# quziyan/NPairLoss

Measured on NVIDIA H100. Metric: N-pair fwd+bwd samples/sec at B=8192,D=512, higher is better.
Workload: dtype f32 (3-pass fp16-split wgmma, f32 accumulate)

## Files before the change

### npairloss_b200/csrc/kernels.cu

```cuda
#include <cassert>
#include <cstdlib>
#include "device.cuh"
#include "kernels.cuh"
#include <cuda.h>

#include <cuda_bf16.h>
#include <cuda_fp16.h>
#include <cfloat>

#include "thresholds.cuh"

namespace npair {
unsigned long long g_kernel_launches = 0;


__device__ __forceinline__ float fast_exp_m2(float sv, float m2) {
  float y;
  asm("ex2.approx.ftz.f32 %0, %1;" : "=f"(y) : "f"(fmaf(sv, LOG2E, -m2)));
  return y;
}

template <bool VEC>
__device__ __forceinline__ float4 load4(const float* __restrict__ x, long long q) {
  if (VEC) return __ldg(reinterpret_cast<const float4*>(x) + q);
  return make_float4(__ldg(x + 4 * q), __ldg(x + 4 * q + 1), __ldg(x + 4 * q + 2), __ldg(x + 4 * q + 3));
}
template <bool VEC>
__device__ __forceinline__ void abs_sum_max(const float* __restrict__ x, long long n, long long t0, long long stride, bool want_max,
                                            float& sum, float& mx) {
  const long long n4 = n >> 2;
  long long i = t0;
  for (; i + 3 * stride < n4; i += 4 * stride) {
    const float4 a = load4<VEC>(x, i), b = load4<VEC>(x, i + stride), c = load4<VEC>(x, i + 2 * stride), d = load4<VEC>(x, i + 3 * stride);
    const float a0 = fabsf(a.x), a1 = fabsf(a.y), a2 = fabsf(a.z), a3 = fabsf(a.w), b0 = fabsf(b.x), b1 = fabsf(b.y), b2 = fabsf(b.z), b3 = fabsf(b.w);
    const float c0 = fabsf(c.x), c1 = fabsf(c.y), c2 = fabsf(c.z), c3 = fabsf(c.w), d0 = fabsf(d.x), d1 = fabsf(d.y), d2 = fabsf(d.z), d3 = fabsf(d.w);
    sum += (a0 + a1) + (a2 + a3) + (b0 + b1) + (b2 + b3) + (c0 + c1) + (c2 + c3) + (d0 + d1) + (d2 + d3);
    if (want_max) {
      mx = fmaxf(mx, fmaxf(fmaxf(fmaxf(a0, a1), fmaxf(a2, a3)), fmaxf(fmaxf(b0, b1), fmaxf(b2, b3))));
      mx = fmaxf(mx, fmaxf(fmaxf(fmaxf(c0, c1), fmaxf(c2, c3)), fmaxf(fmaxf(d0, d1), fmaxf(d2, d3))));
    }
  }
  for (; i < n4; i += stride) {
    const float4 a = load4<VEC>(x, i);
    sum += (fabsf(a.x) + fabsf(a.y)) + (fabsf(a.z) + fabsf(a.w));
    if (want_max) mx = fmaxf(mx, fmaxf(fmaxf(fabsf(a.x), fabsf(a.y)), fmaxf(fabsf(a.z), fabsf(a.w))));
  }
  for (long long j = (n4 << 2) + t0; j < n; j += stride) { sum += fabsf(x[j]); if (want_max) mx = fmaxf(mx, fabsf(x[j])); }
}
template <bool DISJOINT = false>
__device__ __forceinline__ bool prep_reduce_body(const float* __restrict__ xl, long long nl, const float* __restrict__ xt, long long ntot,
                                                 float* __restrict__ partial, int want_scale, RowArrays ra, int Q, BlockScalars* bs) {
  __shared__ float s_sum[8], s_max[8];
  __shared__ int s_last;
  float sum = 0.f, mx = 0.f;
  const long long stride = static_cast<long long>(gridDim.x) * blockDim.x;
  const long long t0 = static_cast<long long>(blockIdx.x) * blockDim.x + threadIdx.x;
  const bool same_range = !DISJOINT && want_scale && xl == xt && nl == ntot;
  const bool local_max = DISJOINT ? want_scale != 0 : same_range;
  if ((reinterpret_cast<uintptr_t>(xl) & 15) == 0) abs_sum_max<true>(xl, nl, t0, stride, local_max, sum, mx);
  else abs_sum_max<false>(xl, nl, t0, stride, local_max, sum, mx);
  if (want_scale && !same_range) {
    if ((reinterpret_cast<uintptr_t>(xt) & 15) == 0) {
      const float4* x4 = reinterpret_cast<const float4*>(xt);
      const long long n4 = ntot >> 2;
      long long i = t0;
      for (; i + 3 * stride < n4; i += 4 * stride) {
        const float4 a = __ldg(x4 + i), b = __ldg(x4 + i + stride), c = __ldg(x4 + i + 2 * stride), d = __ldg(x4 + i + 3 * stride);
        mx = fmaxf(mx, fmaxf(fmaxf(fmaxf(fabsf(a.x), fabsf(a.y)), fmaxf(fabsf(a.z), fabsf(a.w))), fmaxf(fmaxf(fabsf(b.x), fabsf(b.y)), fmaxf(fabsf(b.z), fabsf(b.w)))));
        mx = fmaxf(mx, fmaxf(fmaxf(fmaxf(fabsf(c.x), fabsf(c.y)), fmaxf(fabsf(c.z), fabsf(c.w))), fmaxf(fmaxf(fabsf(d.x), fabsf(d.y)), fmaxf(fabsf(d.z), fabsf(d.w)))));
      }
      for (; i < n4; i += stride) { const float4 a = __ldg(x4 + i); mx = fmaxf(mx, fmaxf(fmaxf(fabsf(a.x), fabsf(a.y)), fmaxf(fabsf(a.z), fabsf(a.w)))); }
      for (long long j = (n4 << 2) + t0; j < ntot; j += stride) mx = fmaxf(mx, fabsf(xt[j]));
    } else {
      for (long long i = t0; i < ntot; i += stride) mx = fmaxf(mx, fabsf(xt[i]));
    }
  }
  for (long long i = t0; i < Q; i += stride) reset_row_stats(ra, i);
  sum = warp_sum(sum); mx = warp_max(mx);
  const int w = threadIdx.x >> 5, l = threadIdx.x & 31;
  if (l == 0) { s_sum[w] = sum; s_max[w] = mx; }
  __syncthreads();
  if (threadIdx.x == 0) {
    sum = 0.f; mx = 0.f;
    for (int k = 0; k < (blockDim.x >> 5); ++k) { sum += s_sum[k]; mx = fmaxf(mx, s_max[k]); }
    partial[blockIdx.x] = sum; partial[1024 + blockIdx.x] = mx;
    __threadfence();
    s_last = (atomicAdd(&bs->ticket0, 1u) == gridDim.x - 1) ? 1 : 0;
  }
  __syncthreads();
  if (!s_last) return false;
  __threadfence();
  __shared__ double s_dsum[8];
  double dsum = 0.0; mx = 0.f;
  for (int b = threadIdx.x; b < static_cast<int>(gridDim.x); b += blockDim.x) { dsum += __ldcg(&partial[b]); mx = fmaxf(mx, __ldcg(&partial[1024 + b])); }
#pragma unroll
  for (int o = 16; o > 0; o >>= 1) { dsum += __shfl_xor_sync(0xffffffffu, dsum, o); mx = fmaxf(mx, __shfl_xor_sync(0xffffffffu, mx, o)); }
  if (l == 0) { s_dsum[w] = dsum; s_max[w] = mx; }
  __syncthreads();
  if (threadIdx.x == 0) {
    dsum = 0.0; mx = 0.f;
    for (int k = 0; k < (blockDim.x >> 5); ++k) { dsum += s_dsum[k]; mx = fmaxf(mx, s_max[k]); }
    bs->asum = static_cast<float>(dsum);
    bs->x_absmax = mx;
    float sc = 1.f, inv = 1.f;
    if (want_scale) { const PreScale ps = pre_scale(mx); sc = ps.scale; inv = ps.inv; }
    bs->x_scale = sc; bs->x_inv_scale = inv;
    bs->err = 0; bs->ticket = 0; bs->ticket2 = 0; bs->ticket0 = 0; bs->ticket3 = 0; bs->sel_active[0] = 0; bs->sel_active[1] = 0;
    bs->cand_n[0] = 0; bs->cand_n[1] = 0;
    bs->n_same = 0; bs->n_diff = 0;
  }
  return true;
}
__global__ void __launch_bounds__(256) prep_reduce_kernel(const float* __restrict__ xl, long long nl, const float* __restrict__ xt, long long ntot,
                                                          float* __restrict__ partial, int want_scale, RowArrays ra, int Q, BlockScalars* bs) {
  prep_reduce_body(xl, nl, xt, ntot, partial, want_scale, ra, Q, bs);
}
void launch_prep_reduce(const float* x_local, long long n_local, const float* x_total, long long n_total, float* partial,
                        int want_scale, RowArrays ra, int Q, BlockScalars* bs, cudaStream_t st) {
  long long nmax = n_local > n_total ? n_local : n_total;
  int nb = static_cast<int>((nmax + 256 * 16 - 1) / (256 * 16));
  if (nb < 1) nb = 1; if (nb > 592) nb = 592;
  prep_reduce_kernel<<<nb, 256, 0, st>>>(x_local, n_local, x_total, n_total, partial, want_scale, ra, Q, bs);
  count_launch();
}
__global__ void __launch_bounds__(256) prep_reduce_memory_kernel(const float* __restrict__ xl, long long nl, const float* __restrict__ xm,
                                                                 long long nm, float* __restrict__ partial, int want_scale, RowArrays ra, int Q,
                                                                 BlockScalars* bs) {
  prep_reduce_body<true>(xl, nl, xm, nm, partial, want_scale, ra, Q, bs);
}
void launch_prep_reduce_memory(const float* x_local, long long n_local, const float* x_mem, long long n_mem, float* partial, int want_scale,
                               RowArrays ra, int Q, BlockScalars* bs, cudaStream_t st) {
  int nb = static_cast<int>((n_local + n_mem + 256 * 16 - 1) / (256 * 16));
  if (nb < 1) nb = 1; if (nb > 592) nb = 592;
  prep_reduce_memory_kernel<<<nb, 256, 0, st>>>(x_local, n_local, x_mem, n_mem, partial, want_scale, ra, Q, bs);
  count_launch();
}

struct SplitArgs {
  const float* x; int N, D;
  uint16_t* Xs; long long ldXs; uint16_t* XsT; long long ldXsT; uint16_t* XlT; long long ldXlT; int row0, Q;
  uint16_t *XcatA, *XcatB; long long Dp;
};
__device__ __forceinline__ void split_load(const SplitArgs& a, int tile_d, int tile_n, float (&v)[8]) {
  const float* __restrict__ x = a.x; const int N = a.N, D = a.D;
  const int t = threadIdx.x, nl = t >> 3, dg = t & 7;
  const int n = tile_n * 32 + nl, d = tile_d * 64 + 8 * dg;
  const bool rowok = n < N;
  if (rowok && d + 7 < D && (D & 3) == 0 && (reinterpret_cast<uintptr_t>(x) & 15) == 0) {
    const float4 a4 = *reinterpret_cast<const float4*>(x + static_cast<long long>(n) * D + d);
    const float4 b4 = *reinterpret_cast<const float4*>(x + static_cast<long long>(n) * D + d + 4);
    v[0] = a4.x; v[1] = a4.y; v[2] = a4.z; v[3] = a4.w; v[4] = b4.x; v[5] = b4.y; v[6] = b4.z; v[7] = b4.w;
  } else {
#pragma unroll
    for (int e = 0; e < 8; ++e) v[e] = (rowok && d + e < D) ? x[static_cast<long long>(n) * D + d + e] : 0.f;
  }
}
template <int PREC>
__device__ __forceinline__ void split_tile(const SplitArgs& a, float sc, int tile_d, int tile_n, const float (&v)[8], int buf) {
  const int N = a.N, D = a.D;
  uint16_t* __restrict__ Xs = a.Xs; const long long ldXs = a.ldXs; uint16_t* __restrict__ XsT = a.XsT; const long long ldXsT = a.ldXsT;
  uint16_t* __restrict__ XlT = a.XlT; const long long ldXlT = a.ldXlT; const int row0 = a.row0, Q = a.Q;
  uint16_t* __restrict__ XcatA = a.XcatA; uint16_t* __restrict__ XcatB = a.XcatB; const long long Dp = a.Dp;
  constexpr int NS = SPLIT_FORMATS[PREC].pieces;
  __shared__ __align__(16) uint16_t tile2[2][NS][64][40];
  uint16_t (*tile)[64][40] = tile2[buf];
  const int n0 = tile_n * 32, d0 = tile_d * 64;
  const int t = threadIdx.x, nl = t >> 3, dg = t & 7;
  const int n = n0 + nl, d = d0 + 8 * dg;
  uint16_t p[8][3];
  uint4 pk[3];
  const bool rowok = n < N;
  split8<PREC>(v, sc, p, pk);
#pragma unroll
  for (int s = 0; s < NS; ++s)
#pragma unroll
    for (int e = 0; e < 8; ++e) tile[s][8 * dg + e][nl] = p[e][s];
  if (rowok && d < Dp && Xs) {
    const long long ps = static_cast<long long>(N) * ldXs;
#pragma unroll
    for (int s = 0; s < NS; ++s) *reinterpret_cast<uint4*>(Xs + s * ps + static_cast<long long>(n) * ldXs + d) = pk[s];
  }
  if (PREC != PREC_BF16 && XcatA && d < Dp) {
    const SimLayout L{NS, Dp};
    if (n < L.padded_rows(N)) store_sim_row<PREC>(XcatB, Dp, n, d, pk, true);
    if (n >= row0 && n < row0 + L.padded_rows(Q)) {
      uint4 pa[3];
#pragma unroll
      for (int s = 0; s < 3; ++s) pa[s] = n < row0 + Q ? pk[s] : make_uint4(0u, 0u, 0u, 0u);
      store_sim_row<PREC>(XcatA, Dp, n - row0, d, pa, false);
    }
  }
  __syncthreads();
  const int dl = t >> 2, nc = t & 3;
  const int dd = d0 + dl, nn = n0 + 8 * nc;
  if (dd < D && nn < N) {
    const long long pt = static_cast<long long>(D) * ldXsT;
    const long long pl = static_cast<long long>(D) * ldXlT;
#pragma unroll
    for (int s = 0; s < NS; ++s) {
      const uint4 q = *reinterpret_cast<const uint4*>(&tile[s][dl][8 * nc]);
      *reinterpret_cast<uint4*>(XsT + s * pt + static_cast<long long>(dd) * ldXsT + nn) = q;
      if (XlT && nn >= row0 && nn < row0 + Q) {
        if (((nn - row0) & 7) == 0 && nn + 8 <= row0 + Q) *reinterpret_cast<uint4*>(XlT + s * pl + static_cast<long long>(dd) * ldXlT + (nn - row0)) = q;
        else
          for (int e = 0; e < 8; ++e)
            if (nn + e < row0 + Q && nn + e < N) XlT[s * pl + static_cast<long long>(dd) * ldXlT + (nn + e - row0)] = tile[s][dl][8 * nc + e];
      } else if (XlT && nn < row0 && nn + 8 > row0) {
        for (int e = 0; e < 8; ++e)
          if (nn + e >= row0 && nn + e < row0 + Q && nn + e < N) XlT[s * pl + static_cast<long long>(dd) * ldXlT + (nn + e - row0)] = tile[s][dl][8 * nc + e];
      }
    }
  }
}
template <int PREC>
__global__ void __launch_bounds__(256) split_kernel(SplitArgs a, const BlockScalars* __restrict__ bs) {
  float v[8];
  split_load(a, blockIdx.x, blockIdx.y, v);
  split_tile<PREC>(a, (PREC == PREC_FP16X2) ? bs->x_scale : 1.f, blockIdx.x, blockIdx.y, v, 0);
}
__device__ __forceinline__ void split_load_memory(const SplitArgs& a, const float* __restrict__ xm, int tile_d, int tile_n, float (&v)[8]) {
  const int N = a.N, D = a.D;
  const int t = threadIdx.x, nl = t >> 3, dg = t & 7;
  const int n = tile_n * 32 + nl, d = tile_d * 64 + 8 * dg;
  const bool rowok = n < N;
  const float* x = n < a.Q ? a.x + static_cast<long long>(n) * D : xm + static_cast<long long>(n - a.Q) * D;
  if (rowok && d + 7 < D && (reinterpret_cast<uintptr_t>(x) & 15) == 0) {
    const float4 a4 = *reinterpret_cast<const float4*>(x + d);
    const float4 b4 = *reinterpret_cast<const float4*>(x + d + 4);
    v[0] = a4.x; v[1] = a4.y; v[2] = a4.z; v[3] = a4.w; v[4] = b4.x; v[5] = b4.y; v[6] = b4.z; v[7] = b4.w;
  } else {
#pragma unroll
    for (int e = 0; e < 8; ++e) v[e] = (rowok && d + e < D) ? x[d + e] : 0.f;
  }
}
template <int PREC>
__global__ void __launch_bounds__(256) split_memory_kernel(SplitArgs a, const float* __restrict__ xm, const BlockScalars* __restrict__ bs) {
  float v[8];
  split_load_memory(a, xm, blockIdx.x, blockIdx.y, v);
  split_tile<PREC>(a, (PREC == PREC_FP16X2) ? bs->x_scale : 1.f, blockIdx.x, blockIdx.y, v, 0);
}
void launch_split_memory(const float* x, int Q, const float* x_mem, int N, int D, int prec, const BlockScalars* bs, uint16_t* Xs,
                         long long ldXs, uint16_t* XsT, long long ldXsT, uint16_t* XcatA, uint16_t* XcatB, long long Dp, cudaStream_t st) {
  dim3 grid((D + 63) / 64, (N + 31) / 32);
  const SplitArgs a{x, N, D, Xs, ldXs, XsT, ldXsT, nullptr, 0, 0, Q, XcatA, XcatB, Dp};
  with_prec(prec, [&](auto P) { split_memory_kernel<P><<<grid, 256, 0, st>>>(a, x_mem, bs); });
  count_launch();
}
__global__ void memory_rows_kernel(const float* __restrict__ label, int Q, const float* __restrict__ mem_label, int m,
                                   float* __restrict__ lab_total, RowRecord* __restrict__ rec) {
  const int stride = gridDim.x * blockDim.x;
  for (int i = blockIdx.x * blockDim.x + threadIdx.x; i < Q + m; i += stride) {
    if (i < Q) { lab_total[i] = label[i]; continue; }
    const float l = mem_label[i - Q];
    lab_total[i] = l;
    rec[i] = RowRecord::memory(l);
  }
}
void launch_memory_rows(const float* label, int Q, const float* mem_label, int m, float* lab_total, RowRecord* rec, cudaStream_t st) {
  const int blocks = (Q + m + 255) / 256;
  memory_rows_kernel<<<blocks < 1024 ? blocks : 1024, 256, 0, st>>>(label, Q, mem_label, m, lab_total, rec);
  count_launch();
}

void launch_split(const float* x_total, int N, int D, int prec, const BlockScalars* bs, uint16_t* Xs, long long ldXs,
                  uint16_t* XsT, long long ldXsT, uint16_t* XlT, long long ldXlT, int row0_local, int Q,
                  uint16_t* XcatA, uint16_t* XcatB, long long Dp, cudaStream_t st) {
  dim3 grid((D + 63) / 64, (N + 31) / 32);
  const SplitArgs a{x_total, N, D, Xs, ldXs, XsT, ldXsT, XlT, ldXlT, row0_local, Q, XcatA, XcatB, Dp};
  with_prec(prec, [&](auto P) { split_kernel<P><<<grid, 256, 0, st>>>(a, bs); });
  count_launch();
}

__global__ void row_stats_ref_kernel(const __grid_constant__ SimRows sim, RowArrays ra) {
  const int i = sim.row0 + blockIdx.x;
  const float li = __ldg(sim.lab_rows + i);
  float minw = FLT_MAX, maxw = -FLT_MAX, maxb = -FLT_MAX, maxall = -FLT_MAX;
  int cnt = 0;
  const float* row = sim.row(i);
  for (int j = threadIdx.x; j < sim.N; j += blockDim.x) {
    if (j == sim.self_col(i)) continue;
    const float v = __ldg(row + j);
    maxall = fmaxf(maxall, v);
    if (__ldg(sim.lab_cols + j) == li) { minw = fminf(minw, v); maxw = fmaxf(maxw, v); ++cnt; } else maxb = fmaxf(maxb, v);
  }
  minw = warp_min(minw); maxw = warp_max(maxw); maxb = warp_max(maxb); maxall = warp_max(maxall); cnt = warp_sum_i(cnt);
  if ((threadIdx.x & 31) == 0) {
    atomicMin(&ra.st_minw[i], f2ord(minw)); atomicMax(&ra.st_maxw[i], f2ord(maxw));
    atomicMax(&ra.st_maxb[i], f2ord(maxb)); atomicMax(&ra.st_maxall[i], f2ord(maxall));
    if (cnt) atomicAdd(&ra.cnt_same[i], cnt);
  }
}
void launch_row_stats_ref(SimRows sim, RowArrays ra, cudaStream_t st) {
  row_stats_ref_kernel<<<sim.rows, 256, 0, st>>>(sim, ra);
  count_launch();
}

__global__ void __launch_bounds__(1024) thresholds_kernel(RowArrays ra, int Q, int N, MiningParams mp, BlockScalars* bs) {
  __shared__ __align__(8) unsigned char scratch[THRESHOLDS_SCRATCH_BYTES];
  thresholds_one_block(ra, Q, N, mp, bs, scratch, nullptr);
}
__global__ void thresholds_world_kernel(const BlockStats* __restrict__ xall, int xstride, int world, long long N, MiningParams mp,
                                        BlockScalars* bs) {
  if (threadIdx.x != 0 || blockIdx.x != 0) return;
  finish_thresholds(xall, world, xstride, static_cast<unsigned long long>(N), N, mp, bs);
}
void launch_thresholds_world(const float* xall, int xstride, int world, long long N, MiningParams mp, BlockScalars* bs, cudaStream_t st) {
  thresholds_world_kernel<<<1, 32, 0, st>>>(reinterpret_cast<const BlockStats*>(xall), xstride, world, N, mp, bs);
  count_launch();
}
void launch_thresholds(RowArrays ra, int Q, int N, MiningParams mp, BlockScalars* bs, cudaStream_t st) {
  thresholds_kernel<<<1, 1024, 0, st>>>(ra, Q, N, mp, bs);
  count_launch();
}

__device__ __forceinline__ float retrieval_cut(float maxw, float max_all, int lane) {
  const float pstar = expf(maxw - max_all);
  if (!(pstar > 0.f)) return -INFINITY;
  uint32_t base = f2ord(maxw), last_ok = base;
  for (int it = 0; it < 8; ++it) {
    const uint32_t kc = base - static_cast<uint32_t>(lane);
    const bool ok = (kc <= base) && (expf(ord2f(kc) - max_all) >= pstar);
    const unsigned bal = __ballot_sync(0xffffffffu, ok);
    const int T = (bal == 0xffffffffu) ? 32 : (__ffs(~bal) - 1);
    if (T > 0) last_ok = base - static_cast<uint32_t>(T - 1);
    if (T < 32) return ord2f(last_ok);
    if (base < 64u) return ord2f(last_ok);
    base -= 32u;
  }
  uint32_t lo = f2ord(-FLT_MAX), hi = last_ok;
  while (lo < hi) {
    const uint32_t mid = lo + ((hi - lo) >> 1);
    if (expf(ord2f(mid) - max_all) >= pstar) hi = mid; else lo = mid + 1u;
  }
  return ord2f(hi);
}

__device__ __forceinline__ float4 ldg_stream(const float4* p) {
  float4 v;
  asm volatile("ld.global.nc.L1::no_allocate.v4.f32 {%0, %1, %2, %3}, [%4];" : "=f"(v.x), "=f"(v.y), "=f"(v.z), "=f"(v.w) : "l"(p));
  return v;
}

__device__ __forceinline__ void lse_elem(float sv, float lab, float li, float scut, float m2, float sgn_p, float thr_p,
                                         float sgn_n, float thr_n, float& A, float& T, int& c) {
  c += (sv >= scut) ? 1 : 0;
  const float e = fast_exp_m2(sv, m2);
  const bool same = (lab == li);
  const float key = sv * (same ? sgn_p : sgn_n);
  const float es = (key <= (same ? thr_p : thr_n)) ? e : 0.f;
  T += es;
  if (same) A += es;
}

__device__ __forceinline__ void publish_tops(const TopSums* recs, int n, long long stride, long long rows, int num_tops, TopsBlock* out,
                                             unsigned int seq) {
  double ls = recs[0].loss_sum, asum = recs[0].asum;
  long long h[3] = {recs[0].hits[0], recs[0].hits[1], recs[0].hits[2]};
  int err = recs[0].err;
  for (int r = 1; r < n; ++r) {
    const TopSums& t = rank_record(recs, stride, r);
    ls += t.loss_sum; h[0] += t.hits[0]; h[1] += t.hits[1]; h[2] += t.hits[2]; asum += t.asum; err |= t.err;
  }
  float tops[5] = {0.f, 0.f, 0.f, 0.f, 0.f};
  tops[0] = static_cast<float>(ls) / static_cast<float>(-rows);
  for (int t = 1; t <= num_tops - 2 && t <= 3; ++t) tops[t] = static_cast<float>(h[t - 1]) / static_cast<float>(rows);
  tops[num_tops - 1] = static_cast<float>(asum) / static_cast<float>(rows);
  for (int t = 0; t < 5; ++t) out->tops[t] = tops[t];
  out->err = err;
  __threadfence_system();
  *reinterpret_cast<volatile unsigned int*>(&out->seq) = seq;
}

__device__ __forceinline__ void lse_finalize_block(int Q, RowArrays ra, BlockScalars* bs, int num_tops, TopsBlock* __restrict__ tops,
                                                   TopSums* __restrict__ xout, unsigned int seq, const float* __restrict__ anchor_w) {
  const int lane = threadIdx.x & 31;
  __shared__ double s_l[8];
  __shared__ int s_h[3][8];
  double ls = 0.0; int h[3] = {0, 0, 0};
  constexpr int FU = 8;
  for (int r0 = threadIdx.x; r0 < Q; r0 += FU * blockDim.x) {
    float lv[FU]; int h0[FU], h1[FU], h2[FU];
#pragma unroll
    for (int u = 0; u < FU; ++u) {
      const int r = r0 + u * blockDim.x;
      const bool ok = r < Q;
      lv[u] = ok ? __ldcg(&ra.logv[r]) : 0.f;
      if (anchor_w) {
        const float wv = ok ? __ldg(&anchor_w[r]) : 0.f;
        lv[u] = wv == 0.f ? 0.f : lv[u] * wv;
      }
      h0[u] = ok ? __ldcg(&ra.hits[r]) : 0; h1[u] = ok ? __ldcg(&ra.hits[Q + r]) : 0; h2[u] = ok ? __ldcg(&ra.hits[2 * Q + r]) : 0;
    }
#pragma unroll
    for (int u = 0; u < FU; ++u) { ls += lv[u]; h[0] += h0[u]; h[1] += h1[u]; h[2] += h2[u]; }
  }
#pragma unroll
  for (int o = 16; o > 0; o >>= 1) {
    ls += __shfl_xor_sync(0xffffffffu, ls, o);
    h[0] += __shfl_xor_sync(0xffffffffu, h[0], o); h[1] += __shfl_xor_sync(0xffffffffu, h[1], o); h[2] += __shfl_xor_sync(0xffffffffu, h[2], o);
  }
  const int w = threadIdx.x >> 5;
  if (lane == 0) { s_l[w] = ls; s_h[0][w] = h[0]; s_h[1][w] = h[1]; s_h[2][w] = h[2]; }
  __syncthreads();
  if (threadIdx.x == 0) {
    TopSums s{0.0, {0, 0, 0}, bs->asum, __ldcg(&bs->err)};
    for (int k = 0; k < (blockDim.x >> 5); ++k) { s.loss_sum += s_l[k]; s.hits[0] += s_h[0][k]; s.hits[1] += s_h[1][k]; s.hits[2] += s_h[2][k]; }
    bs->ticket = 0;
    if (xout) *xout = s;
    else publish_tops(&s, 1, 0, Q, num_tops, tops, seq);
  }
}

#ifndef NPAIR_LSE_U
#define NPAIR_LSE_U 4
#endif
#ifndef NPAIR_LSE_MINB
#define NPAIR_LSE_MINB 3
#endif
__global__ void __launch_bounds__(256, NPAIR_LSE_MINB) lse_rows_kernel(const __grid_constant__ SimRows sim, MiningParams mp, RowArrays ra, BlockScalars* bs,
                                                       int num_tops, TopsBlock* __restrict__ tops,
                                                       float m2c_off , float wscale ,
                                                       TopSums* __restrict__ xout ,
                                                       int wpr ,
                                                       unsigned int seq , int finalize,
                                                       const float* __restrict__ anchor_w , float* __restrict__ row_loss ) {
  const int lane = threadIdx.x & 31;
  __shared__ float s_pA[8], s_pT[8];
  __shared__ int s_pc[8];
#ifndef NPAIR_LSE_REV
#define NPAIR_LSE_REV 1
#endif
  const int blk = NPAIR_LSE_REV ? static_cast<int>(gridDim.x - 1 - blockIdx.x) : static_cast<int>(blockIdx.x);
  const int wib = threadIdx.x >> 5;
  const int il = blk * ((blockDim.x >> 5) / wpr) + wib / wpr;
  const int i = sim.row0 + il;
  const int Q = sim.Q, N = sim.N;
  const float* lab_cols = sim.lab_cols;
  const int part = wib % wpr;
  float A = 0.f, T = 0.f; int c = 0;
  float m2 = 0.f, thr_p = 0.f, thr_n = 0.f, li = 0.f; int cs = 0;
  if (il < sim.rows) {
    constexpr int U = NPAIR_LSE_U;
    const float* row = sim.row(i);
    const int seg = ((N + wpr - 1) / wpr + 128 * U - 1) / (128 * U) * (128 * U);
    const int c_lo = min(N, part * seg), c_hi = min(N, c_lo + seg);
    const int n_full = c_lo + (c_hi - c_lo) / (128 * U) * (128 * U);
    const float4* srow4 = reinterpret_cast<const float4*>(row + c_lo) + lane;
    const float4* lab4 = reinterpret_cast<const float4*>(lab_cols + c_lo) + lane;
    const bool lab_aligned = (reinterpret_cast<uintptr_t>(lab_cols) & 15) == 0;
    const bool fast = lab_aligned && c_lo < n_full;
    float4 v[U], vn[U];
    if (fast) {
#pragma unroll
      for (int u = 0; u < U; ++u) v[u] = ldg_stream(srow4 + 32 * u);
    }
    li = __ldg(sim.lab_rows + i);
    const int self_col = sim.self_col(i);
    const float max_all = ord2f(ra.st_maxall[i]);
    m2 = max_all * LOG2E;
    const float posi = mp.ap_region == REGION_GLOBAL ? bs->posi_global : ra.posi_thr[i];
    const float nega = mp.an_region == REGION_GLOBAL ? bs->nega_global : ra.nega_thr[i];
    if (lane == 0 && part == 0) { ra.posi_thr[i] = posi; ra.nega_thr[i] = nega; }
    const float tp = posi + mp.margin_ident;
    const float tn = nega + mp.margin_diff;
    const float sgn_p = ap_sign(mp.ap_method), sgn_n = an_sign(mp.an_method);
    thr_p = ap_thr(tp, mp.ap_method); thr_n = an_thr(tn, mp.an_method);
    cs = ra.cnt_same[i];
    const float scut = cs > 0 ? retrieval_cut(ord2f(ra.st_maxw[i]), max_all, lane) : INFINITY;
    int base = c_lo;
    if (fast) {
      for (; base < n_full; base += 128 * U, srow4 += 32 * U, lab4 += 32 * U) {
        const bool more = base + 128 * U < n_full;
        if (more) {
#pragma unroll
          for (int u = 0; u < U; ++u) vn[u] = ldg_stream(srow4 + 32 * U + 32 * u);
        }
        float4 l[U];
#pragma unroll
        for (int u = 0; u < U; ++u) l[u] = __ldg(lab4 + 32 * u);
#pragma unroll
        for (int u = 0; u < U; ++u) {
          const int j4 = base + u * 128 + lane * 4;
          const float vv[4] = {v[u].x, v[u].y, v[u].z, v[u].w};
          const float ll[4] = {l[u].x, l[u].y, l[u].z, l[u].w};
          const bool no_self = !sim.self_in4(i, j4);
          if (no_self && ll[0] != li && ll[1] != li && ll[2] != li && ll[3] != li) {
#pragma unroll
            for (int q = 0; q < 4; ++q) {
              c += (vv[q] >= scut) ? 1 : 0;
              const float e = fast_exp_m2(vv[q], m2);
              if (vv[q] * sgn_n <= thr_n) T += e;
            }
          } else if (no_self) {
#pragma unroll
            for (int q = 0; q < 4; ++q) lse_elem(vv[q], ll[q], li, scut, m2, sgn_p, thr_p, sgn_n, thr_n, A, T, c);
          } else {
#pragma unroll
            for (int q = 0; q < 4; ++q)
              if (j4 + q != self_col) lse_elem(vv[q], ll[q], li, scut, m2, sgn_p, thr_p, sgn_n, thr_n, A, T, c);
          }
        }
        if (more) {
#pragma unroll
          for (int u = 0; u < U; ++u) v[u] = vn[u];
        }
      }
    }
    for (; base < c_hi; base += 512) {
#pragma unroll 1
      for (int u = 0; u < 4; ++u) {
        const int j4 = base + u * 128 + lane * 4;
        if (j4 >= c_hi) continue;
        const float4 v4 = *reinterpret_cast<const float4*>(row + j4);
        const float vv[4] = {v4.x, v4.y, v4.z, v4.w};
#pragma unroll
        for (int q = 0; q < 4; ++q)
          if (j4 + q < c_hi && j4 + q != self_col) lse_elem(vv[q], lab_cols[j4 + q], li, scut, m2, sgn_p, thr_p, sgn_n, thr_n, A, T, c);
      }
    }
    A = warp_sum(A); T = warp_sum(T); c = warp_sum_i(c);
  }
  if (wpr > 1) {
    if (lane == 0) { s_pA[wib] = A; s_pT[wib] = T; s_pc[wib] = c; }
    __syncthreads();
    if (part == 0) {
      A = 0.f; T = 0.f; c = 0;
      for (int q = 0; q < wpr; ++q) { A += s_pA[wib + q]; T += s_pT[wib + q]; c += s_pc[wib + q]; }
    }
  }
  if (il < sim.rows && part == 0) {
    if (lane == 0) {
      ra.A[i] = A; ra.T[i] = T;
      const float lv = (A == 0.f || T == 0.f) ? 0.f : logf(A / T);
      ra.logv[i] = lv;
      if (row_loss) row_loss[i] = -lv;
      const int lim = N - 2;
      ra.hits[i] = (cs > 0 && c <= min(1, lim)) ? 1 : 0;
      ra.hits[Q + i] = (cs > 0 && c <= min(5, lim)) ? 1 : 0;
      ra.hits[2 * Q + i] = (cs > 0 && c <= min(10, lim)) ? 1 : 0;
      const float invA = A == 0.f ? 0.f : 1.f / A;
      const float invT = T == 0.f ? 0.f : 1.f / T;
      const float cA = invT - invA;
      const float amin = A > 0.f ? A : T;
      const int j = amin > 0.f ? max(0, ilogbf(wscale) - 127 - ilogbf(amin)) : 0;
      const float fsc = ldexpf(wscale, -j);
      float m2c = T == 0.f ? INFINITY : m2 + log2f(T) + m2c_off;
      float w = 1.f;
      if (anchor_w) {
        w = __ldg(&anchor_w[i]);
        if (!(w >= 0.f && w <= 1.f)) atomicOr(&bs->err, DERR_ANCHOR_WEIGHT);
        m2c = w > 0.f ? m2c - log2f(w) : INFINITY;
      }
      ra.rowrec[i] = RowRecord::make(m2c, thr_n, m2 - static_cast<float>(j), li, thr_p, cA * fsc * w, invT * fsc * w);
    }
  }
  if (!finalize) return;
  __shared__ int s_last;
  __threadfence();
  __syncthreads();
  if (threadIdx.x == 0) s_last = (atomicAdd(&bs->ticket, 1u) == gridDim.x - 1) ? 1 : 0;
  __syncthreads();
  if (!s_last) return;
  __threadfence();
  lse_finalize_block(Q, ra, bs, num_tops, tops, xout, seq, anchor_w);
}
__global__ void lse_finalize_kernel(int Q, RowArrays ra, BlockScalars* bs, int num_tops, TopsBlock* __restrict__ tops, unsigned int seq,
                                    const float* __restrict__ anchor_w) {
  lse_finalize_block(Q, ra, bs, num_tops, tops, nullptr, seq, anchor_w);
}
static void lse_shape(int Q, int N, int* wpr_out, int* threads_out) {
  int wpr = 1;
  while (wpr < 8 && static_cast<long long>(Q) * wpr < 4096 && N / (2 * wpr) >= 512) wpr *= 2;
  if (Q >= 1024 && wpr > 2) wpr = 2;
#ifdef NPAIR_LSE_WPR_FORCE
  wpr = NPAIR_LSE_WPR_FORCE;
#endif
  *wpr_out = wpr;
  if (wpr > 1) { *threads_out = 256; return; }
  int wpb = 8;
  while (wpb > 1 && (Q + wpb - 1) / wpb < 296) wpb >>= 1;
  *threads_out = wpb * 32;
}
void launch_lse_rows(SimRows sim, MiningParams mp, RowArrays ra, BlockScalars* bs, int num_tops, TopsBlock* tops_dev, int world, TopSums* xout,
                     int wlog2, unsigned int seq, bool finalize, AnchorIO aio, cudaStream_t st) {
  int wpr = 1, threads = 256;
  lse_shape(sim.Q, sim.N, &wpr, &threads);
  const int rows_per_blk = threads / 32 / wpr;
  const int grid = (sim.rows + rows_per_blk - 1) / rows_per_blk;
  const float log2_world = xout ? 0.f : log2f(static_cast<float>(world));
  lse_rows_kernel<<<grid, threads, 0, st>>>(sim, mp, ra, bs, num_tops, tops_dev, log2_world - static_cast<float>(wlog2), ldexpf(1.f, wlog2), xout,
                                            wpr, seq, finalize ? 1 : 0, aio.weight, aio.row_loss);
  count_launch();
}
void launch_lse_finalize(int Q, int N, RowArrays ra, BlockScalars* bs, int num_tops, TopsBlock* tops_dev, unsigned int seq, const float* anchor_w,
                         cudaStream_t st) {
  int wpr = 1, threads = 256;
  lse_shape(Q, N, &wpr, &threads);
  lse_finalize_kernel<<<1, threads, 0, st>>>(Q, ra, bs, num_tops, tops_dev, seq, anchor_w);
  count_launch();
}

struct RowScal { float maxall, tp, tn, cA, cT, lab; };
__device__ __forceinline__ RowScal row_scal(const RowRecord* rec, float w) {
  if (!rec) return RowScal{0.f, -INFINITY, -INFINITY, 0.f, 0.f, 0.f};
  const RowRecord r = *rec;
  return RowScal{r.m2(), r.thr_p(), r.thr_n(), r.cA() * w, r.cT() * w, r.label()};
}

__device__ __forceinline__ float gprime(float sv, bool same, const RowScal& r, float sgn_p, float sgn_n) {
  const float e = fast_exp_m2(sv, r.maxall);
  const float key = sv * (same ? sgn_p : sgn_n);
  return (key <= (same ? r.tp : r.tn)) ? e * (same ? r.cA : r.cT) : 0.f;
}

template <int PREC>
__device__ __forceinline__ void store_quad(uint16_t* __restrict__ base, long long piece_stride, long long off, const float g[4]) {
  constexpr int NS = SPLIT_FORMATS[PREC].pieces;
  if (g[0] == 0.f && g[1] == 0.f && g[2] == 0.f && g[3] == 0.f) {
#pragma unroll
    for (int s = 0; s < NS; ++s) *reinterpret_cast<uint2*>(base + s * piece_stride + off) = make_uint2(0u, 0u);
    return;
  }
  uint16_t p[4][3];
#pragma unroll
  for (int e = 0; e < 4; ++e) split3<PREC>(g[e], p[e][0], p[e][1], p[e][2]);
#pragma unroll
  for (int s = 0; s < NS; ++s)
    *reinterpret_cast<uint2*>(base + s * piece_stride + off) =
        make_uint2(static_cast<uint32_t>(p[0][s]) | (static_cast<uint32_t>(p[1][s]) << 16), static_cast<uint32_t>(p[2][s]) | (static_cast<uint32_t>(p[3][s]) << 16));
}

template <int PREC, int MODE>
__global__ void __launch_bounds__(256, 4) build_weights_kernel(const __grid_constant__ SimRows sim, float inv_world, const RowRecord* __restrict__ rs_total,
                                                            MiningParams mp, RowArrays ra,
                                                            uint16_t* __restrict__ H, long long ldH, uint16_t* __restrict__ HT, long long ldHT) {
  constexpr bool SYM = (MODE != BW_SPLIT);
  constexpr int TS = 64;
  const int Q = sim.Q, N = sim.N;
  const int ta = blockIdx.y, tb = blockIdx.x;
  __shared__ RowScal sc_a[TS], sc_b[TS];
  const int a0 = ta * TS, b0 = tb * TS;
  const int t = threadIdx.x, tr = t >> 4, tc = t & 15;
  const float sgn_p = ap_sign(mp.ap_method), sgn_n = an_sign(mp.an_method);
  if (t < TS) {
    sc_a[t] = row_scal(a0 + t < Q ? ra.rowrec + a0 + t : nullptr, 1.f);
  } else if (t < 2 * TS) {
    const int mm = t - TS, m = b0 + mm;
    if (MODE == BW_SYM) {
      sc_b[mm] = row_scal(m < Q ? ra.rowrec + m : nullptr, 1.f);
    } else if (MODE == BW_ROWSCAL) {
      sc_b[mm] = row_scal(m < N ? rs_total + m : nullptr, inv_world);
    } else {
      RowScal r = row_scal(nullptr, 1.f);
      if (m < N) r.lab = sim.lab_cols[m];
      sc_b[mm] = r;
    }
  }
  __syncthreads();
  const int ja0 = a0 + 4 * tr, mb0 = b0 + 4 * tc;
  RowScal rb4[4];
#pragma unroll
  for (int e = 0; e < 4; ++e) rb4[e] = sc_b[4 * tc + e];
  const bool interior = (a0 + TS <= Q) && (b0 + TS <= N) && (sim.self_col(a0) + TS <= b0 || b0 + TS <= sim.self_col(a0));
  const long long psH = static_cast<long long>(Q) * ldH;
  float gT[4][4];
  float4 v4[4];
#pragma unroll
  for (int i = 0; i < 4; ++i) {
    v4[i] = make_float4(0.f, 0.f, 0.f, 0.f);
    if (ja0 + i < Q && mb0 < N) v4[i] = *reinterpret_cast<const float4*>(sim.row(ja0 + i) + mb0);
  }
#pragma unroll
  for (int i = 0; i < 4; ++i) {
    const RowScal rsa = sc_a[4 * tr + i];
    const float sv[4] = {v4[i].x, v4[i].y, v4[i].z, v4[i].w};
    float g[4];
#pragma unroll
    for (int e = 0; e < 4; ++e) {
      const int j = ja0 + i, m = mb0 + e;
      float x = 0.f;
      if (interior || (j < Q && m < N && m != sim.self_col(j))) {
        const bool same = rsa.lab == rb4[e].lab;
        x = gprime(sv[e], same, rsa, sgn_p, sgn_n);
        if (SYM) x += gprime(sv[e], same, rb4[e], sgn_p, sgn_n);
      }
      g[e] = x;
      if (!SYM) gT[e][i] = x;
    }
    if (ja0 + i < Q && mb0 < ldH) store_quad<PREC>(H, psH, static_cast<long long>(ja0 + i) * ldH + mb0, g);
  }
  if (!SYM) {
    const long long psT = static_cast<long long>(N) * ldHT;
#pragma unroll
    for (int e = 0; e < 4; ++e)
      if (mb0 + e < N && ja0 < ldHT) store_quad<PREC>(HT, psT, static_cast<long long>(mb0 + e) * ldHT + ja0, gT[e]);
  }
}
void launch_build_weights(SimRows sim, int world, int mode, const RowRecord* rs_total, MiningParams mp, RowArrays ra, int prec,
                          uint16_t* H, long long ldH, uint16_t* HT, long long ldHT, cudaStream_t st) {
  assert(sim.row0 == 0 && sim.rows == sim.Q && "the weight builder sweeps the rank's whole S");
  dim3 grid((sim.N + 63) / 64, (sim.Q + 63) / 64);
  const float inv_world = 1.f / static_cast<float>(world);
  with_prec(prec, [&](auto P) {
    auto kernel = mode == BW_SYM ? build_weights_kernel<P, BW_SYM> : mode == BW_ROWSCAL ? build_weights_kernel<P, BW_ROWSCAL>
                                                                                        : build_weights_kernel<P, BW_SPLIT>;
    kernel<<<grid, 256, 0, st>>>(sim, inv_world, rs_total, mp, ra, H, ldH, HT, ldHT);
  });
  count_launch();
}

__global__ void __launch_bounds__(256) l2norm_fwd_kernel(const float* __restrict__ x, int rows, int dim, float* __restrict__ y,
                                                         float* __restrict__ inv_norm) {
  const int lane = threadIdx.x & 31;
  const int r = blockIdx.x * (blockDim.x >> 5) + (threadIdx.x >> 5);
  if (r >= rows) return;
  const float* xr = x + static_cast<long long>(r) * dim;
  float* yr = y + static_cast<long long>(r) * dim;
  const bool quad = (dim & 3) == 0;
  const bool vec = quad && ((reinterpret_cast<uintptr_t>(x) | reinterpret_cast<uintptr_t>(y)) & 15) == 0;
  float ss = 0.f;
  if (vec) for (int d = lane * 4; d < dim; d += 128) { const float4 v = *reinterpret_cast<const float4*>(xr + d); ss = fmaf(v.x, v.x, ss); ss = fmaf(v.y, v.y, ss); ss = fmaf(v.z, v.z, ss); ss = fmaf(v.w, v.w, ss); }
  else if (quad) for (int d = lane * 4; d < dim; d += 128) for (int e = 0; e < 4; ++e) ss = fmaf(xr[d + e], xr[d + e], ss);
  else for (int d = lane; d < dim; d += 32) ss = fmaf(xr[d], xr[d], ss);
  ss = warp_sum(ss);
  const float nrm = sqrtf(ss);
  const float inv = nrm > 0.f ? 1.f / nrm : 0.f;
  if (lane == 0 && inv_norm) inv_norm[r] = inv;
  if (vec) for (int d = lane * 4; d < dim; d += 128) {
    const float4 v = *reinterpret_cast<const float4*>(xr + d);
    *reinterpret_cast<float4*>(yr + d) = nrm > 0.f ? make_float4(v.x / nrm, v.y / nrm, v.z / nrm, v.w / nrm) : make_float4(0.f, 0.f, 0.f, 0.f);
  } else for (int d = lane; d < dim; d += 32) yr[d] = nrm > 0.f ? xr[d] / nrm : 0.f;
}
__global__ void __launch_bounds__(256) l2norm_bwd_kernel(const float* __restrict__ y, const float* __restrict__ inv_norm, const float* __restrict__ dy,
                                                         int rows, int dim, float* __restrict__ dx) {
  const int lane = threadIdx.x & 31;
  const int r = blockIdx.x * (blockDim.x >> 5) + (threadIdx.x >> 5);
  if (r >= rows) return;
  const float* yr = y + static_cast<long long>(r) * dim;
  const float* gr = dy + static_cast<long long>(r) * dim;
  float* dr = dx + static_cast<long long>(r) * dim;
  const bool quad = (dim & 3) == 0;
  const bool vec = quad && ((reinterpret_cast<uintptr_t>(y) | reinterpret_cast<uintptr_t>(dy) | reinterpret_cast<uintptr_t>(dx)) & 15) == 0;
  float dot = 0.f;
  if (vec) for (int d = lane * 4; d < dim; d += 128) {
    const float4 a = *reinterpret_cast<const float4*>(yr + d), g = *reinterpret_cast<const float4*>(gr + d);
    dot = fmaf(a.x, g.x, dot); dot = fmaf(a.y, g.y, dot); dot = fmaf(a.z, g.z, dot); dot = fmaf(a.w, g.w, dot);
  } else if (quad) {
    for (int d = lane * 4; d < dim; d += 128) for (int e = 0; e < 4; ++e) dot = fmaf(yr[d + e], gr[d + e], dot);
  } else for (int d = lane; d < dim; d += 32) dot = fmaf(yr[d], gr[d], dot);
  dot = warp_sum(dot);
  const float inv = inv_norm[r];
  if (vec) for (int d = lane * 4; d < dim; d += 128) {
    const float4 a = *reinterpret_cast<const float4*>(yr + d), g = *reinterpret_cast<const float4*>(gr + d);
    *reinterpret_cast<float4*>(dr + d) = make_float4((g.x - a.x * dot) * inv, (g.y - a.y * dot) * inv, (g.z - a.z * dot) * inv, (g.w - a.w * dot) * inv);
  } else for (int d = lane; d < dim; d += 32) dr[d] = (gr[d] - yr[d] * dot) * inv;
}
__global__ void tops_world_kernel(const TopSums* __restrict__ xall, int xstride, int world, long long N, int num_tops, TopsBlock* __restrict__ tops,
                                  unsigned int seq) {
  if (threadIdx.x != 0 || blockIdx.x != 0) return;
  publish_tops(xall, world, xstride, N, num_tops, tops, seq);
}
void launch_tops_world(const float* xall, int xstride, int world, long long N, int num_tops, TopsBlock* tops_dev, unsigned int seq, cudaStream_t st) {
  tops_world_kernel<<<1, 32, 0, st>>>(reinterpret_cast<const TopSums*>(xall), xstride, world, N, num_tops, tops_dev, seq);
  count_launch();
}

__global__ void async_tops_kernel(AsyncWords* __restrict__ aw, int num_tops, float* __restrict__ d_tops) {
  if (threadIdx.x != 0 || blockIdx.x != 0) return;
  const int err = aw->tops.err & (DERR_EMPTY_LIST | DERR_POS_RANGE | DERR_ANCHOR_WEIGHT);
  for (int t = 0; t < 5; ++t) d_tops[t] = err ? __int_as_float(0x7fc00000) : (t < num_tops ? aw->tops.tops[t] : 0.f);
  aw->err |= static_cast<unsigned int>(err);
}
void launch_async_tops(AsyncWords* aw, int num_tops, float* d_tops, cudaStream_t st) {
  async_tops_kernel<<<1, 32, 0, st>>>(aw, num_tops, d_tops);
  count_launch();
}
__global__ void grad_scale_kernel(const float* __restrict__ d_lw, int Q, int wlog2, const BlockScalars* __restrict__ bs,
                                  AsyncWords* __restrict__ aw) {
  if (threadIdx.x != 0 || blockIdx.x != 0) return;
  const float lw_over_q = ldexpf(__fdiv_rn(*d_lw, static_cast<float>(Q)), -wlog2);
  aw->grad_scale = __fmul_rn(__fmul_rn(0.5f, lw_over_q), bs->x_inv_scale);
}
void launch_grad_scale(const float* d_lw, int Q, int wlog2, const BlockScalars* bs, AsyncWords* aw, cudaStream_t st) {
  grad_scale_kernel<<<1, 32, 0, st>>>(d_lw, Q, wlog2, bs, aw);
  count_launch();
}

void launch_l2norm_fwd(const float* x, int rows, int dim, float* y, float* inv_norm, cudaStream_t st) {
  l2norm_fwd_kernel<<<(rows + 7) / 8, 256, 0, st>>>(x, rows, dim, y, inv_norm);
  count_launch();
}
void launch_l2norm_bwd(const float* y, const float* inv_norm, const float* dy, int rows, int dim, float* dx, cudaStream_t st) {
  l2norm_bwd_kernel<<<(rows + 7) / 8, 256, 0, st>>>(y, inv_norm, dy, rows, dim, dx);
  count_launch();
}

}
```

Measured before the change: 10.52 million.

## Overlap split kernel with prep reduction via PDL and batch tiles per block

The prep reduction kernel now signals launch_dependents early, and the split kernel is launched with programmatic stream serialization. Split blocks issue their global loads for several row tiles before griddepcontrol.wait, so input loads overlap the tail of the reduction that produces x_scale. Each block now handles SPLIT_TPB row tiles instead of one, which cuts the block count and raises loads in flight per thread, at the cost of more registers. An inactive probe macro is also added to the LSE rows kernel.

```diff
diff --git a/npairloss_b200/csrc/kernels.cu b/npairloss_b200/csrc/kernels.cu
--- a/npairloss_b200/csrc/kernels.cu
+++ b/npairloss_b200/csrc/kernels.cu
@@ -47,9 +47,13 @@
   }
   for (long long j = (n4 << 2) + t0; j < n; j += stride) { sum += fabsf(x[j]); if (want_max) mx = fmaxf(mx, fabsf(x[j])); }
 }
+#ifndef NPAIR_PREP_PDL
+#define NPAIR_PREP_PDL 1
+#endif
 template <bool DISJOINT = false>
 __device__ __forceinline__ bool prep_reduce_body(const float* __restrict__ xl, long long nl, const float* __restrict__ xt, long long ntot,
                                                  float* __restrict__ partial, int want_scale, RowArrays ra, int Q, BlockScalars* bs) {
+  asm volatile("griddepcontrol.launch_dependents;");
   __shared__ float s_sum[8], s_max[8];
   __shared__ int s_last;
   float sum = 0.f, mx = 0.f;
@@ -212,11 +216,22 @@
     }
   }
 }
+#ifndef NPAIR_SPLIT_TPB
+#define NPAIR_SPLIT_TPB 4
+#endif
+constexpr int SPLIT_TPB = NPAIR_SPLIT_TPB;
 template <int PREC>
 __global__ void __launch_bounds__(256) split_kernel(SplitArgs a, const BlockScalars* __restrict__ bs) {
-  float v[8];
-  split_load(a, blockIdx.x, blockIdx.y, v);
-  split_tile<PREC>(a, (PREC == PREC_FP16X2) ? bs->x_scale : 1.f, blockIdx.x, blockIdx.y, v, 0);
+  const int n_tiles = (a.N + 31) / 32, t0 = blockIdx.y * SPLIT_TPB;
+  float v[SPLIT_TPB][8];
+#pragma unroll
+  for (int k = 0; k < SPLIT_TPB; ++k)
+    if (t0 + k < n_tiles) split_load(a, blockIdx.x, t0 + k, v[k]);
+  asm volatile("griddepcontrol.wait;" ::: "memory");
+  const float sc = (PREC == PREC_FP16X2) ? bs->x_scale : 1.f;
+#pragma unroll
+  for (int k = 0; k < SPLIT_TPB; ++k)
+    if (t0 + k < n_tiles) split_tile<PREC>(a, sc, blockIdx.x, t0 + k, v[k], k & 1);
 }
 __device__ __forceinline__ void split_load_memory(const SplitArgs& a, const float* __restrict__ xm, int tile_d, int tile_n, float (&v)[8]) {
   const int N = a.N, D = a.D;
@@ -265,9 +280,17 @@
 void launch_split(const float* x_total, int N, int D, int prec, const BlockScalars* bs, uint16_t* Xs, long long ldXs,
                   uint16_t* XsT, long long ldXsT, uint16_t* XlT, long long ldXlT, int row0_local, int Q,
                   uint16_t* XcatA, uint16_t* XcatB, long long Dp, cudaStream_t st) {
-  dim3 grid((D + 63) / 64, (N + 31) / 32);
+  const int n_tiles = (N + 31) / 32;
   const SplitArgs a{x_total, N, D, Xs, ldXs, XsT, ldXsT, XlT, ldXlT, row0_local, Q, XcatA, XcatB, Dp};
-  with_prec(prec, [&](auto P) { split_kernel<P><<<grid, 256, 0, st>>>(a, bs); });
+  cudaLaunchConfig_t cfg = {};
+  cfg.gridDim = dim3((D + 63) / 64, (n_tiles + SPLIT_TPB - 1) / SPLIT_TPB);
+  cfg.blockDim = dim3(256);
+  cfg.stream = st;
+  cudaLaunchAttribute attr[1];
+  attr[0].id = cudaLaunchAttributeProgrammaticStreamSerialization;
+  attr[0].val.programmaticStreamSerializationAllowed = NPAIR_PREP_PDL;
+  cfg.attrs = attr; cfg.numAttrs = 1;
+  with_prec(prec, [&](auto P) { cudaLaunchKernelEx(&cfg, split_kernel<P>, a, bs); });
   count_launch();
 }
 
@@ -416,6 +439,9 @@
 #endif
 #ifndef NPAIR_LSE_MINB
 #define NPAIR_LSE_MINB 3
+#endif
+#ifndef NPAIR_ROWS_PROBE
+#define NPAIR_ROWS_PROBE 0
 #endif
 __global__ void __launch_bounds__(256, NPAIR_LSE_MINB) lse_rows_kernel(const __grid_constant__ SimRows sim, MiningParams mp, RowArrays ra, BlockScalars* bs,
                                                        int num_tops, TopsBlock* __restrict__ tops,
@@ -466,7 +492,11 @@
     const float sgn_p = ap_sign(mp.ap_method), sgn_n = an_sign(mp.an_method);
     thr_p = ap_thr(tp, mp.ap_method); thr_n = an_thr(tn, mp.an_method);
     cs = ra.cnt_same[i];
+#if NPAIR_ROWS_PROBE == 1
+    const float scut = INFINITY;
+#else
     const float scut = cs > 0 ? retrieval_cut(ord2f(ra.st_maxw[i]), max_all, lane) : INFINITY;
+#endif
     int base = c_lo;
     if (fast) {
       for (; base < n_full; base += 128 * U, srow4 += 32 * U, lab4 += 32 * U) {
@@ -475,6 +505,10 @@
 #pragma unroll
           for (int u = 0; u < U; ++u) vn[u] = ldg_stream(srow4 + 32 * U + 32 * u);
         }
+#if NPAIR_ROWS_PROBE == 1
+#pragma unroll
+        for (int u = 0; u < U; ++u) T += (v[u].x + v[u].y) + (v[u].z + v[u].w);
+#else
         float4 l[U];
 #pragma unroll
         for (int u = 0; u < U; ++u) l[u] = __ldg(lab4 + 32 * u);
@@ -500,6 +534,7 @@
               if (j4 + q != self_col) lse_elem(vv[q], ll[q], li, scut, m2, sgn_p, thr_p, sgn_n, thr_n, A, T, c);
           }
         }
+#endif
         if (more) {
 #pragma unroll
           for (int u = 0; u < U; ++u) v[u] = vn[u];
@@ -554,7 +589,7 @@
       ra.rowrec[i] = RowRecord::make(m2c, thr_n, m2 - static_cast<float>(j), li, thr_p, cA * fsc * w, invT * fsc * w);
     }
   }
-  if (!finalize) return;
+  if (!finalize || NPAIR_ROWS_PROBE == 2) return;
   __shared__ int s_last;
   __threadfence();
   __syncthreads();
```

Result: no change. 10.57 million (median of 6 runs) (+0.5%).
